# bluenote-1577/skani

Measured on AMD Instinct MI355X. Metric: genome-pairs/sec (triangle, ~5 Mbp genomes), higher is better.
Workload: dtype u64

## Files before the change

### skani_amd/csrc/capi.hip

```cpp
#include <algorithm>
#include <cmath>
#include <cstdlib>
#include <new>

#include "internal.h"

using namespace skh;

namespace {

template <class F> int guarded(skh_ctx* ctx, F&& f) {
    try {
        if (ctx) { PinScope scope(ctx->device, &ctx->ring); if (!ctx->pending_sorts.empty()) reap_pending_sorts(ctx); f(); } else f();
        return SKH_OK;
    }
    catch (const std::bad_alloc&) { if (ctx) ctx->err = "out of host memory"; return SKH_ERR_NOMEM; }
    catch (const PeerError& e) { if (ctx) ctx->err = e.what(); return SKH_ERR_PEER; }
    catch (const Error& e) { if (ctx) ctx->err = e.what(); return SKH_ERR_DEVICE; }
    catch (const std::invalid_argument& e) { if (ctx) ctx->err = e.what(); return SKH_ERR_INVALID; }
    catch (const std::exception& e) { if (ctx) ctx->err = e.what(); return SKH_ERR_INTERNAL; }
    catch (...) { if (ctx) ctx->err = "unknown error"; return SKH_ERR_INTERNAL; }
}

void check_params(const skh_sketch_params* p) {
// ... 38 lines not shown
    skh_ctx* ctx = new (std::nothrow) skh_ctx();
    if (!ctx) return SKH_ERR_NOMEM;
    int rc = guarded(ctx, [&] {
        dev_open(device, &ctx->stream, &ctx->stream2);
        ctx->device = device; ctx->ring.s0 = ctx->stream; ctx->ring.s1 = ctx->stream2;
        ctx->scan_ticket.alloc(2); dzero(ctx->scan_ticket.p, 8, ctx->stream); dsync(ctx->stream);
        auto env = [](const char* n, uint64_t dflt) { const char* v = getenv(n); return v && *v ? (uint64_t)strtoull(v, nullptr, 10) : dflt; };
        ctx->tune.seed_scratch_bytes = env("SKH_TUNE_SEED_SCRATCH_BYTES", ctx->tune.seed_scratch_bytes); ctx->tune.seed_scratch_fixed = getenv("SKH_TUNE_SEED_SCRATCH_BYTES") != nullptr;
        ctx->tune.seed_tile_cap = (uint32_t)env("SKH_TUNE_SEED_TILE_CAP", ctx->tune.seed_tile_cap);
        ctx->tune.screen_cells = env("SKH_TUNE_SCREEN_CELLS", ctx->tune.screen_cells);
        ctx->tune.chain_anchors = env("SKH_TUNE_CHAIN_ANCHORS", ctx->tune.chain_anchors);
        ctx->tune.chain_super_tiles = (uint32_t)env("SKH_TUNE_CHAIN_SUPER_TILES", ctx->tune.chain_super_tiles);
        ctx->tune.chain_dp_lds_slots = (uint32_t)env("SKH_TUNE_CHAIN_DP_LDS_SLOTS", ctx->tune.chain_dp_lds_slots);
        ctx->tune.build_match_cap = (uint32_t)env("SKH_TUNE_BUILD_MATCH_CAP", ctx->tune.build_match_cap);
        ctx->tune.marker_lds_max = (uint32_t)env("SKH_TUNE_MARKER_LDS_MAX", ctx->tune.marker_lds_max);
        ctx->tune.build_slice_max = (uint32_t)env("SKH_TUNE_BUILD_SLICE_MAX", ctx->tune.build_slice_max);
        ctx->tune.join_bitmap_words = (uint32_t)env("SKH_TUNE_JOIN_BITMAP_WORDS", ctx->tune.join_bitmap_words);
        ctx->tune.screen_planes = (uint32_t)env("SKH_TUNE_SCREEN_PLANES", ctx->tune.screen_planes);
        ctx->tune.screen_count_rows = (uint32_t)env("SKH_TUNE_SCREEN_COUNT_ROWS", ctx->tune.screen_count_rows);
        ctx->tune.screen_col_order = (uint32_t)env("SKH_TUNE_SCREEN_COL_ORDER", ctx->tune.screen_col_order);
        ctx->tune.marker_gate = (uint32_t)env("SKH_TUNE_MARKER_GATE", ctx->tune.marker_gate);
        ctx->tune.screen_cells_dense = (uint32_t)env("SKH_TUNE_SCREEN_CELLS_DENSE", 0);
        ctx->tune.build_resalt_all = (uint32_t)env("SKH_TUNE_BUILD_RESALT_ALL", 0);
        ctx->tune.screen_sort_radix = (uint32_t)env("SKH_TUNE_SCREEN_SORT_RADIX", 0);
        ctx->tune.skeys_avg = (uint32_t)env("SKH_TUNE_SKEYS_AVG", ctx->tune.skeys_avg);
        ctx->tune.skeys_cap = (uint32_t)env("SKH_TUNE_SKEYS_CAP", 0);
        ctx->tune.wide_sweep_dp = (uint32_t)env("SKH_TUNE_WIDE_SWEEP_DP", 0);
        ctx->tune.scan_one_max = env("SKH_TUNE_SCAN_ONE_MAX", ctx->tune.scan_one_max); ctx->tune.scan_two_max = env("SKH_TUNE_SCAN_TWO_MAX", ctx->tune.scan_two_max);
        ctx->tune.dist_fail = (uint32_t)env("SKH_TUNE_DIST_FAIL", 0);
        ctx->tune.dist_key_range_w1 = (uint32_t)env("SKH_TUNE_DIST_KEY_RANGE_W1", 0);
        ctx->tune.greedy_big_min = (uint32_t)env("SKH_TUNE_GREEDY_BIG_MIN", ctx->tune.greedy_big_min);
        ctx->tune.wide_span = std::min<uint64_t>(ctx->tune.wide_span, env("SKH_TUNE_WIDE_SPAN", ctx->tune.wide_span));
        ctx->tune.greedy_len_limit = (uint32_t)std::min<uint64_t>(0x10000, env("SKH_TUNE_GREEDY_LEN_LIMIT", 0x10000));
    });
    if (rc != SKH_OK) { delete ctx; return rc; }
    *out = ctx;
    return SKH_OK;
}

void skh_ctx_destroy(skh_ctx* ctx) {
    if (!ctx) return;
    dev_drain(ctx->device, ctx->stream, ctx->stream2);
    ctx->arena.release_all();
    ctx->model_c125 = GbdtModel(); ctx->model_c200 = GbdtModel(); ctx->scan_ticket.release(); ctx->part_cnt.release();
    dcache_trim();
    dev_close(ctx->stream, ctx->stream2);
    delete ctx;
}

const char* skh_last_error(const skh_ctx* ctx) { return ctx ? ctx->err.c_str() : "null context"; }
int skh_device_memory(uint64_t* live_bytes, uint64_t* idle_bytes, int trim) {
    try {
        if (trim) dcache_trim();
        size_t live = 0, idle = 0; dcache_stats(&live, &idle);
        if (live_bytes) *live_bytes = live;
        if (idle_bytes) *idle_bytes = idle;
        return SKH_OK;
    } catch (...) { return SKH_ERR_INTERNAL; }
}
void skh_free(void* p) { free(p); }

int skh_load_models(skh_ctx* ctx, const char* p125, const char* p200) {
    if (!ctx || !p125 || !p200) return SKH_ERR_INVALID;
    return guarded(ctx, [&] { load_model(ctx, p125, ctx->model_c125); load_model(ctx, p200, ctx->model_c200); });
}

int skh_genomes_pack(skh_ctx* ctx, const uint8_t* bases, const uint64_t* contig_off, const uint32_t* contig_genome, uint32_t n_contigs,
                     uint32_t n_genomes, int on_device, int seeding_mode, skh_genome_set** out) {
    if (!ctx || !out || (n_contigs && (!bases || !contig_off || !contig_genome))) return SKH_ERR_INVALID;
    *out = nullptr;
    skh_genome_set* gs = nullptr;
    int rc = guarded(ctx, [&] {
        if (seeding_mode != SKH_SEED_SCALAR && seeding_mode != SKH_SEED_AVX2) throw std::invalid_argument("bad seeding_mode");
        gs = new skh_genome_set();
        gs->ctx = ctx; gs->seeding_mode = seeding_mode;
        std::vector<uint64_t> len(n_contigs);
        for (uint32_t i = 0; i < n_contigs; i++) {
// ... 501 lines not shown
```

### skani_amd/csrc/chain.hip

```cpp
#include <algorithm>
#include <cmath>

#include "internal.h"

namespace skh {

#include "chain_types.h"
#include "chain_join.h"
#include "chain_chunk.h"
#include "chain_dp.h"
#include "chain_select.h"
#include "chain_stats.h"
#include "chain_estimate.h"

namespace {

static void genome_halves(const skh_sketch_set* S) {
    std::lock_guard<std::mutex> lk(S->cache_mu);
    if (S->halves.size() == S->n_genomes && S->n_genomes) return;
    S->halves.resize(S->n_genomes);
    for (uint32_t g = 0; g < S->n_genomes; g++) {
        skh_sketch_set::GenomeHalf& h = S->halves[g];
        h.n_pos = (uint32_t)(S->pos_off[g + 1] - S->pos_off[g]); h.pos0 = (uint32_t)S->pos_off[g];
        h.seed = S->p_seed.p + S->pos_off[g]; h.g = S->p_g.p + S->pos_off[g]; h.rep = S->p_rep.p; h.salt = S->salt[g];
// ... 301 lines not shown
                check_launch("chain_dp");
                SKH_LAUNCH(interval_emit_kernel<W>, (NC + 3) / 4, 256, 0, ctx->stream, NC, (const Chunk*)chunks, (const unsigned long long*)best,
                           (const uint32_t*)chunk_pair, ec);
                check_launch("interval_emit");
            }
        }
        if (!stage_filled) fill_regions(ctx, stage_fills);
#define SKH_GREEDY(CAP) SKH_LAUNCH(greedy_fast_kernel<CAP>, np, 64, 0, ctx->stream, np, (const uint32_t*)g_order, (const uint32_t*)d_pi0, (const uint32_t*)d_pc0, \
                   (const uint32_t*)ivl_cnt, (const Interval*)ivls, ctx->tune.greedy_len_limit, big_min, ivl_next, chunk_head, n_acc); check_launch("greedy_fast")
        tr.mark("dp (+order sort)");
        uint32_t* g_keys = ctx->arena.get<uint32_t>(np); uint32_t* g_order = ctx->arena.get<uint32_t>(np);
        if (np <= GREEDY_ORDER_ONE_MAX) {
            SKH_LAUNCH(greedy_order_kernel, 1u, 1024, 0, ctx->stream, np, (const uint32_t*)ivl_cnt, g_order);
            check_launch("greedy_order");
        } else {
            SKH_LAUNCH(greedy_order_keys_kernel, (np + 255) / 256, 256, 0, ctx->stream, np, (const uint32_t*)ivl_cnt, g_keys, g_order);
            check_launch("greedy_order_keys");
            sort_pairs_u32_u32(ctx, g_keys, g_order, np, 16);
        }
        SKH_GREEDY(256); SKH_GREEDY(512); SKH_GREEDY(1024);
#undef SKH_GREEDY
        SKH_LAUNCH(greedy_kernel, (np + 3) / 4, 256, 0, ctx->stream, np, (const uint32_t*)d_pi0, (const uint32_t*)d_pc0,
                   (const uint32_t*)ivl_cnt, (const Interval*)ivls, big_min, ivl_next, chunk_head, n_acc);
        check_launch("greedy");
        if (NS) {
            SKH_LAUNCH(greedy_big_kernel, np, 1024, 0, ctx->stream, np, (const uint32_t*)d_pi0, (const uint32_t*)d_ps0, (const uint32_t*)d_pc0,
                       (const uint32_t*)ivl_cnt, (const Interval*)ivls, big_min, greedy_scratch, ivl_next, chunk_head, n_acc);
            check_launch("greedy_big");
        }
        tr.mark("greedy");
        double* chunk_est = ctx->arena.get<double>(NC + 1); uint32_t* chunk_w = ctx->arena.get<uint32_t>(NC + 1);
        uint4* chunk_sums = ctx->arena.get<uint4>(NC + 1);
        if (NC) {
            SKH_LAUNCH(chunk_stats_kernel<W>, (NC + 255) / 256, 256, 0, ctx->stream, NC, (const Chunk*)chunks, (const uint32_t*)chunk_pair, (const uint32_t*)chunk_head,
                       (const uint32_t*)ivl_next, (const Interval*)ivls, d_pairs, d_wide, (const unsigned long long*)imk, c, k, chunk_est, chunk_w, chunk_sums);
            check_launch("chunk_stats");
        }
        tr.mark("chunk_stats");
        FinalizeArgs fa{};
        fa.n_pairs = np; fa.c = c; fa.k = k; fa.min_af = mp.min_af; fa.both_min_af = mp.both_min_af; fa.robust = mp.robust; fa.median = mp.median;
        fa.learned = model ? 1 : 0; fa.compute_ci = mp.compute_ci;
        if (model) { fa.nodes = model->nodes.p; fa.tree_off = model->off.p; fa.n_trees = model->n_trees; fa.shrinkage = model->shrinkage; fa.bias = model->bias; }
        FinalizeScratch fs{ctx->arena.get<double>(NC + 1), ctx->arena.get<double>(NC + 1), ctx->arena.get<uint32_t>(NC + 1), ctx->arena.get<uint32_t>(NC + 1),
                           ctx->arena.get<uint64_t>(NC + 1)};
        uint32_t* n_est = ctx->arena.get<uint32_t>(np);
#define SKH_FIN(CAP, MIN, MAX, THR) SKH_LAUNCH((finalize_kernel<CAP, MIN, MAX, THR>), np, THR, 0, ctx->stream, fa, d_pairs, (const uint32_t*)d_pc0, (const uint32_t*)n_chunks, \
                   (const double*)chunk_est, (const uint32_t*)chunk_w, (const uint4*)chunk_sums, fs, n_est, d_out + p0); \
        check_launch("finalize")
        bool any_mid = false, any_long = false;
        for (uint32_t i = 0; i < np && !any_long; i++) { any_mid = any_mid || pc0[i + 1] - pc0[i] > 320; any_long = pc0[i + 1] - pc0[i] > 1024; }
        SKH_FIN(320, 0, 320, FIN_THREADS);
        if (any_mid) { SKH_FIN(1024, 321, 1024, FIN_THREADS); }
        if (any_long) { SKH_FIN(1, 1025, 0xFFFFFFFFu, 1024); }
#undef SKH_FIN
        tr.mark("finalize");
        if (stats) {
            std::vector<uint32_t> h_nc(np), h_ni(np), h_nacc(np), h_ne(np);
            d2h(h_nc.data(), n_chunks, np * 4, ctx->stream); d2h(h_ni.data(), ivl_cnt, np * 4, ctx->stream);
            d2h(h_nacc.data(), n_acc, np * 4, ctx->stream); d2h(h_ne.data(), n_est, np * 4, ctx->stream);
            std::vector<Co> hanc((size_t)NA), hanr((size_t)NA);
            d2h(hanc.data(), anc_q, (uint64_t)NA * sizeof(Co), ctx->stream); d2h(hanr.data(), anc_r, (uint64_t)NA * sizeof(Co), ctx->stream);
            for (uint32_t i = 0; i < np; i++) {
                skh_chain_stats& st = stats[p0 + i];
                const uint32_t an = std::min(pair_anch[p0 + i], pa0[i + 1] - pa0[i]);
                st.switched = (pds[p0 + i].flags >> 2) & 1u; st.n_chunks = h_nc[i]; st.n_intervals = h_ni[i]; st.n_accepted = h_nacc[i]; st.n_estimates = h_ne[i];
                st.reserved = 0; st.n_anchors = pair_anch[p0 + i]; st.n_qpos = pair_inq[p0 + i];
                if constexpr (W::wide) st.anchor_checksum = an ? fnv_anchors(hanc, hanr, pa0[i], pa0[i] + an, job.host_go_a64[p0 + i], pds[p0 + i].a_nctg, job.host_go_b64[p0 + i], pds[p0 + i].b_nctg) : 0;
                else st.anchor_checksum = an ? fnv_anchors(hanc, hanr, pa0[i], pa0[i] + an, job.host_go_a[p0 + i], pds[p0 + i].a_nctg, job.host_go_b[p0 + i], pds[p0 + i].b_nctg) : 0;
                if (pair_anch[p0 + i] == 0) { st.switched = 1; st.n_qpos = 0; }
            }
        }
        if (ctx->pin_results.holds(out + p0)) d2h_pinned(out + p0, d_out + p0, (size_t)np * sizeof(skh_ani_result), ctx->stream);
        else d2h(out + p0, d_out + p0, (size_t)np * sizeof(skh_ani_result), ctx->stream);
        ctx->arena.rewind(arena_mark);
        p0 = p1;
        }
        ctx->arena.rewind(super_mark);
        sp0 = sp1;
    }
    uint32_t h_err = 0;
    d2h(&h_err, d_err, 4, ctx->stream);
    tr.mark("results d2h");
    if (h_err) throw Error("internal capacity bound violated in chain pipeline (" + std::to_string(h_err) + " events)");
}

}

// ... 118 lines not shown
```

### skani_amd/csrc/chain_estimate.h

```cpp
#pragma once

__device__ __forceinline__ double wave_sum_f64(double v) {
#pragma unroll
    for (int d = 32; d > 0; d >>= 1) v += __shfl_xor(v, d, 64);
    return v;
}
__device__ __forceinline__ uint64_t wave_sum_u64(uint64_t v) {
#pragma unroll
    for (int d = 32; d > 0; d >>= 1) v += __shfl_xor(v, d, 64);
    return v;
}

struct FinalizeArgs {
    uint32_t n_pairs, c, k;
    double min_af, both_min_af; int robust, median, learned, compute_ci;
    const GbdtModel::Node* nodes; const uint32_t* tree_off; uint32_t n_trees; float shrinkage, bias;
};
struct FinalizeScratch { double *u_est, *s_est; uint32_t *u_w, *s_w; uint64_t* cum; };

constexpr uint64_t WYRAND_STEP = 0xA0761D6478BD642Full;
__device__ __forceinline__ uint64_t wyrand_mix(uint64_t s) {
    const uint64_t b = s ^ 0xE7037ED1A0B428DBull;
    const uint32_t s0 = (uint32_t)s, s1 = (uint32_t)(s >> 32), b0 = (uint32_t)b, b1 = (uint32_t)(b >> 32);
    const uint64_t p00 = (uint64_t)s0 * b0;
    const uint64_t p01 = (uint64_t)s0 * b1 + (p00 >> 32);
    const uint64_t p10 = (uint64_t)s1 * b0 + (uint32_t)p01;
    const uint64_t p11 = (uint64_t)s1 * b1 + (p01 >> 32) + (p10 >> 32);
    return ((p10 << 32) | (uint32_t)p00) ^ p11;
}
__device__ __forceinline__ uint64_t wyrand_state(uint64_t d) { return 7ull + (d + 1ull) * WYRAND_STEP; }
__device__ __forceinline__ uint64_t wyrand_draw(uint64_t d) { return wyrand_mix(wyrand_state(d)); }

constexpr uint32_t FIN_WAVES = 2, FIN_THREADS = 64 * FIN_WAVES;
template <uint32_t FIN_LDS, uint32_t FIN_MIN, uint32_t FIN_MAX, uint32_t THREADS>
__global__ __launch_bounds__(THREADS) void finalize_kernel(FinalizeArgs fa, const PairDesc* pairs, const uint32_t* pc0, const uint32_t* n_chunks,
                                                       const double* chunk_est, const uint32_t* chunk_w, const uint4* chunk_sums, FinalizeScratch fs,
                                                       uint32_t* n_est_out, skh_ani_result* out) {
    __shared__ double lds_boot[128];
    __shared__ double lds_u[FIN_LDS], lds_s[FIN_LDS];
    __shared__ uint64_t lds_cum[FIN_LDS];
    __shared__ uint32_t lds_uw[FIN_LDS], lds_sw[FIN_LDS];
    __shared__ uint32_t lds_hdr[4];
    __shared__ uint64_t lds_total;
    const uint32_t wv = threadIdx.x >> 6, tid = threadIdx.x;
    const uint32_t p = blockIdx.x;
    if (p >= fa.n_pairs) return;
    const uint32_t l = lane_id();
    const PairDesc pd = pairs[p];
    const uint32_t C0 = pc0[p], nc = n_chunks[p];
    if (nc < FIN_MIN || nc > FIN_MAX) return;
    constexpr uint32_t WAVES = THREADS / 64;
    const bool in_lds = nc <= FIN_LDS;
    double* U = in_lds ? lds_u : fs.u_est + C0; uint32_t* UW = in_lds ? lds_uw : fs.u_w + C0;
    double* S = in_lds ? lds_s : fs.s_est + C0; uint32_t* SW = in_lds ? lds_sw : fs.s_w + C0;
    uint64_t* CUM = in_lds ? lds_cum : fs.cum + C0;
    if (wv == 0) {
        uint32_t n = 0, acl = 0, nchains = 0, tqb = 0;
        for (uint32_t b = 0; b < nc; b += 64) {
            const uint32_t s = C0 + b + l;
            if (b + l < nc) { const uint4 cs = chunk_sums[s]; acl += cs.x; nchains += cs.y; tqb += cs.z; }
            const bool v = b + l < nc && chunk_w[s] != NONE;
            const unsigned long long m = __ballot(v);
            if (v) { const uint32_t o = n + (uint32_t)__popcll(m & ((1ull << l) - 1ull)); U[o] = chunk_est[s]; UW[o] = chunk_w[s]; }
            n += (uint32_t)__popcll(m);
        }
        acl = wave_sum(acl); nchains = wave_sum(nchains); tqb = wave_sum(tqb);
        if (l == 0) { n_est_out[p] = n; lds_hdr[0] = n; lds_hdr[1] = acl; lds_hdr[2] = nchains; lds_hdr[3] = tqb; }
    }
    __syncthreads();
    const uint32_t n = lds_hdr[0], acl = lds_hdr[1], nchains = lds_hdr[2], tqb = lds_hdr[3];
// ... 59 lines not shown
        const uint64_t cv = i < n ? CUM[i] : 0;
        const unsigned long long mlo = __ballot(i < n && cv >= thr_lo), mhi = __ballot(i < n && cv >= thr_hi);
        if (lower_i == n && mlo) lower_i = b + (uint32_t)__ffsll((long long)mlo) - 1u;
        if (upper_i == n && mhi) upper_i = b + (uint32_t)__ffsll((long long)mhi) - 1u;
    }
    if (lower_i == n) lower_i = 0;
    upper_i = upper_i == n ? n - 1 : upper_i + 1;
    double wsum = 0., esum = 0.; uint64_t tm = 0;
    for (uint32_t i = l; i < n; i += 64) {
        const double e = S[i]; esum += e;
        if (i >= lower_i && i < upper_i) { wsum += e * (double)SW[i]; tm += SW[i]; }
    }
    wsum = wave_sum_f64(wsum); esum = wave_sum_f64(esum); tm = wave_sum_u64(tm);
    double final_ani = wsum / (double)tm;
    const double mean = esum / (double)n;
    double var = 0.;
    for (uint32_t i = l; i < n; i += 64) { const double d = mean - S[i]; var += d * d; }
    var = wave_sum_f64(var);
    const double sd = sqrt(var / (double)n);
    double ci_lo = 0., ci_hi = 1.;
    if (fa.compute_ci && n >= 10) {
        uint32_t nsteps = 0; while ((1u << nsteps) < n) nsteps++;
        auto search64 = [&](uint64_t x) { uint32_t lo = 0, hi = n - 1; for (uint32_t st = 0; st < nsteps; st++) { const uint32_t mid = (lo + hi) >> 1; const bool gt = CUM[mid] > x; hi = gt ? mid : hi; lo = gt ? lo : mid + 1; } return lo; };
        if (in_lds && total_mult < 0xFFFFFFFFull) {
            uint32_t* C32 = UW; uint32_t* T = (uint32_t*)U;
            uint32_t sh = 0; while ((total_mult >> sh) >= 512) sh++;
            const uint32_t nb = (uint32_t)(total_mult >> sh) + 1;
            for (uint32_t i = tid; i < n; i += THREADS) C32[i] = (uint32_t)CUM[i];
            for (uint32_t b = tid; b < nb; b += THREADS) T[b] = search64((uint64_t)b << sh) | (search64((uint64_t)(b + 1) << sh) << 16);
            __syncthreads();
            const uint32_t tot32 = (uint32_t)total_mult;
            const uint64_t step_it = (uint64_t)n * WYRAND_STEP, step_256 = 256ull * WYRAND_STEP;
            for (uint32_t it0 = 4 * wv; it0 < 100; it0 += 4 * WAVES) {
              uint64_t st[4];
#pragma unroll
              for (int u = 0; u < 4; u++) st[u] = wyrand_state((uint64_t)it0 * n + (uint64_t)l + 64u * (uint32_t)u);
              double sg[4];
#pragma unroll
              for (int g = 0; g < 4; g++) {
                double s = 0.;
                uint64_t sm[4];
#pragma unroll
                for (int u = 0; u < 4; u++) { sm[u] = st[u]; st[u] += step_it; }
                for (uint32_t j0 = l; j0 < n; j0 += 256) {
                    uint32_t x[4], lo[4], hi[4]; bool on[4];
#pragma unroll
                    for (int u = 0; u < 4; u++) {
                        const uint32_t j = j0 + 64u * (uint32_t)u;
                        on[u] = j < n;
                        const uint64_t r = wyrand_mix(sm[u]); sm[u] += step_256;
                        x[u] = (uint32_t)(((uint64_t)(uint32_t)(r >> 32) * tot32 + __umulhi((uint32_t)r, tot32)) >> 32);
                        const uint32_t tb = T[x[u] >> sh];
                        lo[u] = tb & 0xFFFFu; hi[u] = tb >> 16;
                    }
#pragma unroll
                    for (int u = 0; u < 4; u++) {
                        while (lo[u] < hi[u]) { const uint32_t mid = (lo[u] + hi[u]) >> 1; const bool gt = C32[mid] > x[u]; hi[u] = gt ? mid : hi[u]; lo[u] = gt ? lo[u] : mid + 1; }
                    }
#pragma unroll
                    for (int u = 0; u < 4; u++) if (on[u]) s += S[lo[u]];
                }
                sg[g] = s;
              }
#pragma unroll
              for (int d = 32; d > 0; d >>= 1) {
#pragma unroll
                  for (int g = 0; g < 4; g++) sg[g] += __shfl_xor(sg[g], d, 64);
              }
              if (l == 0) {
#pragma unroll
                  for (int g = 0; g < 4; g++) lds_boot[it0 + g] = sg[g] / (double)n;
              }
            }
        } else {
            for (uint32_t it = wv; it < 100; it += WAVES) {
                double s = 0.;
                for (uint32_t j0 = l; j0 < n; j0 += 64) {
                    const uint64_t r = wyrand_draw((uint64_t)it * n + j0);
                    s += S[search64(__umul64hi(r, total_mult))];
                }
                s = wave_sum_f64(s);
                if (l == 0) lds_boot[it] = s / (double)n;
            }
// ... 57 lines not shown
```

### skani_amd/csrc/chain_stats.h

```cpp
#pragma once

constexpr int STATS_REG = 4;

template <class W>
__global__ __launch_bounds__(256) void chunk_stats_kernel(uint32_t n_slots, const Chunk* chunks, const uint32_t* chunk_pair, const uint32_t* chunk_head,
                                                          const uint32_t* ivl_next, const Interval* ivls, const PairDesc* pairs, const WidePair* wide, const unsigned long long* inq_mask,
                                                          uint32_t c, uint32_t k, double* chunk_est, uint32_t* chunk_w, uint4* chunk_sums) {
    using Co = typename W::Co; using Arr = typename W::Arr;
    const uint32_t slot = blockIdx.x * blockDim.x + threadIdx.x;
    const uint32_t l = lane_id();
    const bool valid = slot < n_slots;
    const uint32_t head = valid ? chunk_head[slot] : NONE;
    if (valid) chunk_w[slot] = NONE;
    uint32_t total_anchors = 0, rq0 = 0xFFFFFFFFu, rq1 = 0, tbcq = 0, sum_len = 0, n_int = 0, s_begin = 0, s_end = 0; Co qoff = 0;
    uint32_t lo[STATS_REG], hi[STATS_REG];
#pragma unroll
    for (int i = 0; i < STATS_REG; i++) { lo[i] = 1; hi[i] = 0; }
    bool active = false;
    const void* ag = nullptr; uint32_t ag64 = 0; const unsigned long long* mk = nullptr;
    if (head != NONE) {
        const Chunk ck = chunks[slot];
        const uint32_t p = chunk_pair[slot];
        const bool switched = (pairs[p].flags & 4u) != 0;
        mk = inq_mask + (uint64_t)pairs[p].tile0 * (JOIN_TILE / 64);
        s_begin = ck.s_begin; s_end = ck.s_end;
        if constexpr (W::wide) { const CoArr a = wide[p].a_g; ag = a.p; ag64 = a.is64; qoff = wide[p].a_goff[ck.qctg]; }
        else { ag = pairs[p].a_g; qoff = ck.qoff; }
        for (uint32_t e = head; e != NONE; e = ivl_next[e]) {
            const Interval iv = ivls[e];
            total_anchors += iv.na;
            if (iv.q0 < rq0) rq0 = iv.q0;
            if (iv.q1 > rq1) rq1 = iv.q1;
            tbcq += (switched ? iv.r1 - iv.r0 : iv.q1 - iv.q0) + k + 2 * c;
            sum_len += (iv.q1 - iv.q0) + 2 * c + k;
            const uint32_t l0 = iv.q0 > c ? iv.q0 - c : 0, h0 = iv.q1 + c;
#pragma unroll
            for (int i = 0; i < STATS_REG; i++) if (n_int == (uint32_t)i) { lo[i] = l0; hi[i] = h0; }
            n_int++;
        }
        const bool sensitive = c < 200;
        active = rq1 - rq0 >= MIN_LENGTH_COVER;
        chunk_sums[slot] = make_uint4(sum_len, n_int, sensitive ? sum_len : (active ? rq1 - rq0 + 2 * c + k : 0u), 0u);
    } else if (valid) chunk_sums[slot] = make_uint4(0, 0, 0, 0);
    uint32_t in_u = 0, in_range = 0, in_list = 0;
    unsigned long long todo = __ballot(active);
    constexpr int PF = 4;
    struct Raw { Co v; unsigned long long m; };
    Raw cur[PF] = {}, nxt[PF] = {};
    auto fetch = [&](const Arr& ag_j, const unsigned long long* mk_j, uint32_t s2, uint32_t se_j) -> Raw {
        const uint32_t s = s2 < se_j ? s2 : (se_j ? se_j - 1u : 0u);
        const unsigned long long m = global_of(mk_j)[((s >> 8) << 2) | (s & 3u)];
        return Raw{(Co)ag_j[s], m};
    };
    auto value = [](const Raw& r, uint32_t s2, uint32_t se_j) -> Co {
        return s2 < se_j ? (r.v & ~(Co)1) | (Co)((r.m >> ((s2 >> 2) & 63u)) & 1ull) : (Co)0;
    };
    auto bcast_arr = [&](int src) -> Arr {
        const unsigned long long v = (unsigned long long)ag;
        const uint32_t lo32 = wave_readlane((uint32_t)v, src), hi32 = wave_readlane((uint32_t)(v >> 32), src);
        const void* ptr = (const void*)(((unsigned long long)hi32 << 32) | lo32);
        if constexpr (W::wide) return CoArr{ptr, wave_readlane(ag64, src)}; else return global_of((const uint32_t*)ptr);
    };
    auto bcast_ptr = [&](const void* ptr, int src) -> const void* {
        const unsigned long long v = (unsigned long long)ptr;
        const uint32_t lo32 = wave_readlane((uint32_t)v, src), hi32 = wave_readlane((uint32_t)(v >> 32), src);
        return (const void*)(((unsigned long long)hi32 << 32) | lo32);
    };
    int j = -1; uint32_t sb = 0, se = 0;
    Arr agj{}; const unsigned long long* mkj = nullptr;
    if (todo) {
        j = __ffsll((long long)todo) - 1; todo &= todo - 1ull;
        sb = wave_readlane(s_begin, j); se = wave_readlane(s_end, j);
        agj = bcast_arr(j); mkj = (const unsigned long long*)bcast_ptr(mk, j);
#pragma unroll
        for (int u = 0; u < PF; u++) cur[u] = fetch(agj, mkj, sb + 64u * (uint32_t)u + l, se);
    }
    while (j >= 0) {
        const bool more = todo != 0;
        const int jn = more ? __ffsll((long long)todo) - 1 : j;
        todo &= todo - 1ull;
        const uint32_t sbn = wave_readlane(s_begin, jn), sen = wave_readlane(s_end, jn);
        const Arr agn = bcast_arr(jn); const unsigned long long* mkn = (const unsigned long long*)bcast_ptr(mk, jn);
#pragma unroll
        for (int u = 0; u < PF; u++) nxt[u] = fetch(agn, mkn, sbn + 64u * (uint32_t)u + l, sen);
        const uint32_t nj = wave_readlane(n_int, j), q0j = wave_readlane(rq0, j), q1j = wave_readlane(rq1, j), headj = wave_readlane(head, j);
        const Co qoffj = wave_readlane(qoff, j);
        uint32_t lj[STATS_REG], wj[STATS_REG];
#pragma unroll
        for (int i = 0; i < STATS_REG; i++) { lj[i] = 0; wj[i] = 0; if (i == 0 || (uint32_t)i < nj) { lj[i] = wave_readlane(lo[i], j); wj[i] = wave_readlane(hi[i], j) - lj[i]; } }
        const uint32_t qwj = q1j - q0j;
        uint32_t cu = 0, cr = 0, cl = 0;
        auto count = [&](Co v) {
            const bool on = (v & 1u) != 0;
            const uint32_t pos = (uint32_t)((v >> 1) - qoffj);
            bool hit;
            if (nj <= (uint32_t)STATS_REG) {
                hit = pos - lj[0] <= wj[0];
                if (nj > 1) { hit = hit || pos - lj[1] <= wj[1]; if (nj > 2) { hit = hit || pos - lj[2] <= wj[2]; if (nj > 3) hit = hit || pos - lj[3] <= wj[3]; } }
            } else {
                hit = false;
                for (uint32_t e = headj; e != NONE; e = ivl_next[e]) { const Interval iv = ivls[e]; const uint32_t l0 = iv.q0 > c ? iv.q0 - c : 0; hit = hit || (pos >= l0 && pos <= iv.q1 + c); }
            }
            cl += (uint32_t)__popcll(__ballot(on));
            cu += (uint32_t)__popcll(__ballot(on && hit));
            cr += (uint32_t)__popcll(__ballot(on && pos - q0j <= qwj));
        };
#pragma unroll
        for (int u = 0; u < PF; u++) if (sb + 64u * (uint32_t)u < se) count(value(cur[u], sb + 64u * (uint32_t)u + l, se));
        for (uint32_t b2 = sb + 64u * PF; b2 < se; b2 += 64) count(value(fetch(agj, mkj, b2 + l, se), b2 + l, se));
        if ((int)l == j) { in_u = cu; in_range = cr; in_list = cl; }
        j = more ? jn : -1; sb = sbn; se = sen; agj = agn; mkj = mkn;
#pragma unroll
        for (int u = 0; u < PF; u++) cur[u] = nxt[u];
    }
    if (!active) return;
    uint32_t considered = in_list;
    const double inv_k = 1. / (double)k;
    const double putative = pow((double)total_anchors / (double)in_u, inv_k);
    if (putative > 0.950 && tbcq > c * 4 && rq1 - rq0 < CHUNK_SIZE * 9 / 10 && (double)considered > 1.05 * (double)in_range)
        considered = in_range;
    double ml = (double)total_anchors / (double)considered;
    if (!(ml < 1.)) ml = 1.;
    chunk_est[slot] = pow(ml, inv_k); chunk_w[slot] = considered;
}
```

### skani_amd/csrc/internal.h

```cpp
#pragma once
#include <chrono>
#include <functional>
#include <mutex>
#include <memory>
#include <string>
#include <vector>

#include "../../include/skani_hip.h"
#include "common.h"

namespace skh {

struct Arena {
    struct Chunk { char* p; size_t cap, off; };
    std::vector<Chunk> chunks;
    size_t min_chunk = (size_t)256 << 20;
    ~Arena() { for (auto& c : chunks) dfree(c.p); }
    void* take(size_t bytes) {
        bytes = (bytes + 255) & ~(size_t)255;
        for (auto& c : chunks) if (c.cap - c.off >= bytes) { void* r = c.p + c.off; c.off += bytes; return r; }
        size_t cap = bytes > min_chunk ? bytes : min_chunk;
        Chunk c{(char*)dmalloc(cap), cap, bytes};
        chunks.push_back(c);
        return c.p;
// ... 19 lines not shown
    DBuf<uint32_t> off; DBuf<Node> nodes;
    bool loaded() const { return n_trees != 0; }
};

}

struct skh_tunables {
    uint64_t seed_scratch_bytes = (uint64_t)16 << 30;
    bool seed_scratch_fixed = false;
    uint32_t seed_tile_cap = 0;
    uint64_t screen_cells = (uint64_t)2 << 30;
    uint64_t chain_anchors = (uint64_t)512 << 20;
    uint32_t chain_super_tiles = 1u << 20;
    uint32_t wide_sweep_dp = 0;
    uint32_t build_resalt_all = 0;
    uint32_t screen_sort_radix = 0;
    uint32_t skeys_avg = 1400;
    uint32_t skeys_cap = 0;
    uint32_t screen_cells_dense = 0;
    uint32_t screen_count_rows = 1;
    uint32_t screen_col_order = 1;
    uint32_t marker_gate = 1;
    uint32_t screen_planes = 8;
    uint32_t join_bitmap_words = 8192;
    uint32_t build_slice_max = 0;
    uint32_t marker_lds_max = 0;
    uint32_t build_match_cap = 0;
    uint32_t greedy_len_limit = 0x10000;
    uint32_t greedy_big_min = 2049;
    uint64_t scan_one_max = ~0ull, scan_two_max = ~0ull;
    uint32_t dist_key_range_w1 = 0;
    uint32_t dist_fail = 0;
    uint32_t chain_dp_lds_slots = 8;
    uint64_t wide_span = (1ull << 31) - 8192;
};

namespace skh {
struct PendingSort {
    DBuf<uint64_t> raw; DBuf<char> tmp; DevEvent ev; std::mutex mu;
    DBuf<uint32_t> mat; DBuf<uint64_t> work; DBuf<char> sort_tmp;
    void release() { std::lock_guard<std::mutex> lk(mu); raw.release(); tmp.release(); mat.release(); work.release(); sort_tmp.release(); }
};
}

struct skh_ctx {
    skh_tunables tune;
    int device = 0;
    devStream_t stream{};
    devStream_t stream2{};
    std::string err;
    skh::Arena arena;
    skh::GbdtModel model_c125, model_c200;
    skh_timings timings{};
    skh::PinBuf pin_pairs;
    skh::PinBuf pin_results;
    skh::PinRing ring;
    skh::DBuf<uint32_t> scan_ticket;
    bool screen_planes_checked = false;
    skh::DBuf<uint32_t> part_cnt; bool part_cnt_clean = false;
    std::vector<std::shared_ptr<skh::PendingSort>> pending_sorts;
};

namespace skh { struct Transport; }
struct skh_comm { skh::Transport* t = nullptr; ~skh_comm(); };

struct skh_genome_set {
    skh_ctx* ctx = nullptr;
    int seeding_mode = 0;
    uint32_t n_genomes = 0, n_contigs = 0;
    uint64_t n_words = 0, total_bases = 0;
    std::vector<skh::ContigDesc> contigs;
    std::vector<uint64_t> genome_contig_off;
    skh::DBuf<uint32_t> packed;
    skh::DBuf<uint32_t> nmask;
    skh::DBuf<skh::ContigDesc> d_contigs;
    std::vector<skh::SeedTile> tiles;
    std::vector<uint32_t> genome_first_tile;
    std::vector<uint32_t> tile_cached_for;
    skh::DBuf<skh::SeedTile> d_tiles;
    skh::DBuf<uint32_t> d_genome_first_tile;
    bool open = false; uint64_t cap_units = 0, n_units = 0; uint32_t cap_contigs = 0, n_batches = 0;
    skh::DBuf<uint8_t> stage[2];
    std::vector<std::shared_ptr<skh::DevEvent>> copied;
    std::mutex copied_mu;
};

struct skh_sketch_set {
    skh_ctx* ctx = nullptr;
    skh_sketch_params params{};
// ... 163 lines not shown
```

Before: 41.31 million.

## Count chunk stats via binary search and popcount; cache bootstrap draws in table

The chunk stats kernel gets a new default path. Each active lane finds the query-range and interval boundaries in its own sorted anchor list with galloping and binary searches, then counts marked anchors by popcounting mask words. This replaces the wave-cooperative streaming scan over every anchor, which remains available behind a tunable. Separately, the finalize bootstrap can read precomputed wyrand draws from a device table built once per context instead of hashing each draw, trading ALU work for global loads.

```diff
diff --git a/skani_amd/csrc/capi.hip b/skani_amd/csrc/capi.hip
--- a/skani_amd/csrc/capi.hip
+++ b/skani_amd/csrc/capi.hip
@@ -94,6 +94,8 @@
         ctx->tune.greedy_big_min = (uint32_t)env("SKH_TUNE_GREEDY_BIG_MIN", ctx->tune.greedy_big_min);
         ctx->tune.wide_span = std::min<uint64_t>(ctx->tune.wide_span, env("SKH_TUNE_WIDE_SPAN", ctx->tune.wide_span));
         ctx->tune.greedy_len_limit = (uint32_t)std::min<uint64_t>(0x10000, env("SKH_TUNE_GREEDY_LEN_LIMIT", 0x10000));
+        ctx->tune.stats_stream = (uint32_t)env("SKH_TUNE_STATS_STREAM", ctx->tune.stats_stream);
+        ctx->tune.boot_table = (uint32_t)env("SKH_TUNE_BOOT_TABLE", ctx->tune.boot_table);
     });
     if (rc != SKH_OK) { delete ctx; return rc; }
     *out = ctx;
@@ -104,7 +106,7 @@
     if (!ctx) return;
     dev_drain(ctx->device, ctx->stream, ctx->stream2);
     ctx->arena.release_all();
-    ctx->model_c125 = GbdtModel(); ctx->model_c200 = GbdtModel(); ctx->scan_ticket.release(); ctx->part_cnt.release();
+    ctx->model_c125 = GbdtModel(); ctx->model_c200 = GbdtModel(); ctx->scan_ticket.release(); ctx->part_cnt.release(); ctx->boot_draws.release();
     dcache_trim();
     dev_close(ctx->stream, ctx->stream2);
     delete ctx;
diff --git a/skani_amd/csrc/chain.hip b/skani_amd/csrc/chain.hip
--- a/skani_amd/csrc/chain.hip
+++ b/skani_amd/csrc/chain.hip
@@ -357,8 +357,10 @@
         double* chunk_est = ctx->arena.get<double>(NC + 1); uint32_t* chunk_w = ctx->arena.get<uint32_t>(NC + 1);
         uint4* chunk_sums = ctx->arena.get<uint4>(NC + 1);
         if (NC) {
-            SKH_LAUNCH(chunk_stats_kernel<W>, (NC + 255) / 256, 256, 0, ctx->stream, NC, (const Chunk*)chunks, (const uint32_t*)chunk_pair, (const uint32_t*)chunk_head,
-                       (const uint32_t*)ivl_next, (const Interval*)ivls, d_pairs, d_wide, (const unsigned long long*)imk, c, k, chunk_est, chunk_w, chunk_sums);
+#define SKH_STATS(STREAM) SKH_LAUNCH((chunk_stats_kernel<W, STREAM>), (NC + 255) / 256, 256, 0, ctx->stream, NC, (const Chunk*)chunks, (const uint32_t*)chunk_pair, (const uint32_t*)chunk_head, \
+                       (const uint32_t*)ivl_next, (const Interval*)ivls, d_pairs, d_wide, (const unsigned long long*)imk, c, k, chunk_est, chunk_w, chunk_sums)
+            if (ctx->tune.stats_stream) { SKH_STATS(true); } else { SKH_STATS(false); }
+#undef SKH_STATS
             check_launch("chunk_stats");
         }
         tr.mark("chunk_stats");
@@ -369,8 +371,14 @@
         FinalizeScratch fs{ctx->arena.get<double>(NC + 1), ctx->arena.get<double>(NC + 1), ctx->arena.get<uint32_t>(NC + 1), ctx->arena.get<uint32_t>(NC + 1),
                            ctx->arena.get<uint64_t>(NC + 1)};
         uint32_t* n_est = ctx->arena.get<uint32_t>(np);
-#define SKH_FIN(CAP, MIN, MAX, THR) SKH_LAUNCH((finalize_kernel<CAP, MIN, MAX, THR>), np, THR, 0, ctx->stream, fa, d_pairs, (const uint32_t*)d_pc0, (const uint32_t*)n_chunks, \
-                   (const double*)chunk_est, (const uint32_t*)chunk_w, (const uint4*)chunk_sums, fs, n_est, d_out + p0); \
+        if (ctx->tune.boot_table && fa.compute_ci && !ctx->boot_draws.p) {
+            ctx->boot_draws.alloc(BOOT_DRAWS);
+            SKH_LAUNCH(boot_draws_kernel, (BOOT_DRAWS + 255) / 256, 256, 0, ctx->stream, BOOT_DRAWS, ctx->boot_draws.p); check_launch("boot_draws");
+        }
+        const uint64_t* draws = ctx->tune.boot_table ? ctx->boot_draws.p : nullptr;
+#define SKH_FIN_T(CAP, MIN, MAX, THR, TAB) SKH_LAUNCH((finalize_kernel<CAP, MIN, MAX, THR, TAB>), np, THR, 0, ctx->stream, fa, d_pairs, (const uint32_t*)d_pc0, (const uint32_t*)n_chunks, \
+                   (const double*)chunk_est, (const uint32_t*)chunk_w, (const uint4*)chunk_sums, fs, draws, n_est, d_out + p0)
+#define SKH_FIN(CAP, MIN, MAX, THR) if (draws && CAP > 1) { SKH_FIN_T(CAP, MIN, MAX, THR, (CAP > 1)); } else { SKH_FIN_T(CAP, MIN, MAX, THR, false); } \
         check_launch("finalize")
         bool any_mid = false, any_long = false;
         for (uint32_t i = 0; i < np && !any_long; i++) { any_mid = any_mid || pc0[i + 1] - pc0[i] > 320; any_long = pc0[i + 1] - pc0[i] > 1024; }
@@ -378,6 +386,7 @@
         if (any_mid) { SKH_FIN(1024, 321, 1024, FIN_THREADS); }
         if (any_long) { SKH_FIN(1, 1025, 0xFFFFFFFFu, 1024); }
 #undef SKH_FIN
+#undef SKH_FIN_T
         tr.mark("finalize");
         if (stats) {
             std::vector<uint32_t> h_nc(np), h_ni(np), h_nacc(np), h_ne(np);
diff --git a/skani_amd/csrc/chain_estimate.h b/skani_amd/csrc/chain_estimate.h
--- a/skani_amd/csrc/chain_estimate.h
+++ b/skani_amd/csrc/chain_estimate.h
@@ -30,12 +30,18 @@
 }
 __device__ __forceinline__ uint64_t wyrand_state(uint64_t d) { return 7ull + (d + 1ull) * WYRAND_STEP; }
 __device__ __forceinline__ uint64_t wyrand_draw(uint64_t d) { return wyrand_mix(wyrand_state(d)); }
+constexpr uint32_t BOOT_RESAMPLES = 100, FIN_LDS_MAX = 1024, BOOT_DRAWS = BOOT_RESAMPLES * FIN_LDS_MAX;
+__global__ __launch_bounds__(256) void boot_draws_kernel(uint32_t n, uint64_t* table) {
+    const uint32_t d = blockIdx.x * blockDim.x + threadIdx.x;
+    if (d < n) table[d] = wyrand_draw(d);
+}
 
 constexpr uint32_t FIN_WAVES = 2, FIN_THREADS = 64 * FIN_WAVES;
-template <uint32_t FIN_LDS, uint32_t FIN_MIN, uint32_t FIN_MAX, uint32_t THREADS>
+template <uint32_t FIN_LDS, uint32_t FIN_MIN, uint32_t FIN_MAX, uint32_t THREADS, bool TABLE>
 __global__ __launch_bounds__(THREADS) void finalize_kernel(FinalizeArgs fa, const PairDesc* pairs, const uint32_t* pc0, const uint32_t* n_chunks,
                                                        const double* chunk_est, const uint32_t* chunk_w, const uint4* chunk_sums, FinalizeScratch fs,
-                                                       uint32_t* n_est_out, skh_ani_result* out) {
+                                                       const uint64_t* draws, uint32_t* n_est_out, skh_ani_result* out) {
+    static_assert(!TABLE || BOOT_RESAMPLES * FIN_LDS <= BOOT_DRAWS, "the draw table covers 100 resamples of the largest LDS instantiation");
     __shared__ double lds_boot[128];
     __shared__ double lds_u[FIN_LDS], lds_s[FIN_LDS];
     __shared__ uint64_t lds_cum[FIN_LDS];
@@ -161,9 +167,12 @@
             const uint32_t tot32 = (uint32_t)total_mult;
             const uint64_t step_it = (uint64_t)n * WYRAND_STEP, step_256 = 256ull * WYRAND_STEP;
             for (uint32_t it0 = 4 * wv; it0 < 100; it0 += 4 * WAVES) {
-              uint64_t st[4];
-#pragma unroll
-              for (int u = 0; u < 4; u++) st[u] = wyrand_state((uint64_t)it0 * n + (uint64_t)l + 64u * (uint32_t)u);
+              uint64_t st[4] = {};
+              if constexpr (!TABLE) {
+#pragma unroll
+                for (int u = 0; u < 4; u++) st[u] = wyrand_state((uint64_t)it0 * n + (uint64_t)l + 64u * (uint32_t)u);
+              }
+              const GlobalPtr<uint64_t> tab = global_of(draws);
               double sg[4];
 #pragma unroll
               for (int g = 0; g < 4; g++) {
@@ -171,13 +180,16 @@
                 uint64_t sm[4];
 #pragma unroll
                 for (int u = 0; u < 4; u++) { sm[u] = st[u]; st[u] += step_it; }
+                const uint32_t d0 = (it0 + (uint32_t)g) * n;
                 for (uint32_t j0 = l; j0 < n; j0 += 256) {
                     uint32_t x[4], lo[4], hi[4]; bool on[4];
 #pragma unroll
                     for (int u = 0; u < 4; u++) {
                         const uint32_t j = j0 + 64u * (uint32_t)u;
                         on[u] = j < n;
-                        const uint64_t r = wyrand_mix(sm[u]); sm[u] += step_256;
+                        uint64_t r;
+                        if constexpr (TABLE) r = on[u] ? tab[d0 + j] : 0ull;
+                        else { r = wyrand_mix(sm[u]); sm[u] += step_256; }
                         x[u] = (uint32_t)(((uint64_t)(uint32_t)(r >> 32) * tot32 + __umulhi((uint32_t)r, tot32)) >> 32);
                         const uint32_t tb = T[x[u] >> sh];
                         lo[u] = tb & 0xFFFFu; hi[u] = tb >> 16;
diff --git a/skani_amd/csrc/chain_stats.h b/skani_amd/csrc/chain_stats.h
--- a/skani_amd/csrc/chain_stats.h
+++ b/skani_amd/csrc/chain_stats.h
@@ -2,7 +2,7 @@
 
 constexpr int STATS_REG = 4;
 
-template <class W>
+template <class W, bool STREAM>
 __global__ __launch_bounds__(256) void chunk_stats_kernel(uint32_t n_slots, const Chunk* chunks, const uint32_t* chunk_pair, const uint32_t* chunk_head,
                                                           const uint32_t* ivl_next, const Interval* ivls, const PairDesc* pairs, const WidePair* wide, const unsigned long long* inq_mask,
                                                           uint32_t c, uint32_t k, double* chunk_est, uint32_t* chunk_w, uint4* chunk_sums) {
@@ -43,75 +43,168 @@
         chunk_sums[slot] = make_uint4(sum_len, n_int, sensitive ? sum_len : (active ? rq1 - rq0 + 2 * c + k : 0u), 0u);
     } else if (valid) chunk_sums[slot] = make_uint4(0, 0, 0, 0);
     uint32_t in_u = 0, in_range = 0, in_list = 0;
-    unsigned long long todo = __ballot(active);
-    constexpr int PF = 4;
-    struct Raw { Co v; unsigned long long m; };
-    Raw cur[PF] = {}, nxt[PF] = {};
-    auto fetch = [&](const Arr& ag_j, const unsigned long long* mk_j, uint32_t s2, uint32_t se_j) -> Raw {
-        const uint32_t s = s2 < se_j ? s2 : (se_j ? se_j - 1u : 0u);
-        const unsigned long long m = global_of(mk_j)[((s >> 8) << 2) | (s & 3u)];
-        return Raw{(Co)ag_j[s], m};
-    };
-    auto value = [](const Raw& r, uint32_t s2, uint32_t se_j) -> Co {
-        return s2 < se_j ? (r.v & ~(Co)1) | (Co)((r.m >> ((s2 >> 2) & 63u)) & 1ull) : (Co)0;
-    };
-    auto bcast_arr = [&](int src) -> Arr {
-        const unsigned long long v = (unsigned long long)ag;
-        const uint32_t lo32 = wave_readlane((uint32_t)v, src), hi32 = wave_readlane((uint32_t)(v >> 32), src);
-        const void* ptr = (const void*)(((unsigned long long)hi32 << 32) | lo32);
-        if constexpr (W::wide) return CoArr{ptr, wave_readlane(ag64, src)}; else return global_of((const uint32_t*)ptr);
-    };
-    auto bcast_ptr = [&](const void* ptr, int src) -> const void* {
-        const unsigned long long v = (unsigned long long)ptr;
-        const uint32_t lo32 = wave_readlane((uint32_t)v, src), hi32 = wave_readlane((uint32_t)(v >> 32), src);
-        return (const void*)(((unsigned long long)hi32 << 32) | lo32);
-    };
-    int j = -1; uint32_t sb = 0, se = 0;
-    Arr agj{}; const unsigned long long* mkj = nullptr;
-    if (todo) {
-        j = __ffsll((long long)todo) - 1; todo &= todo - 1ull;
-        sb = wave_readlane(s_begin, j); se = wave_readlane(s_end, j);
-        agj = bcast_arr(j); mkj = (const unsigned long long*)bcast_ptr(mk, j);
-#pragma unroll
-        for (int u = 0; u < PF; u++) cur[u] = fetch(agj, mkj, sb + 64u * (uint32_t)u + l, se);
-    }
-    while (j >= 0) {
-        const bool more = todo != 0;
-        const int jn = more ? __ffsll((long long)todo) - 1 : j;
-        todo &= todo - 1ull;
-        const uint32_t sbn = wave_readlane(s_begin, jn), sen = wave_readlane(s_end, jn);
-        const Arr agn = bcast_arr(jn); const unsigned long long* mkn = (const unsigned long long*)bcast_ptr(mk, jn);
-#pragma unroll
-        for (int u = 0; u < PF; u++) nxt[u] = fetch(agn, mkn, sbn + 64u * (uint32_t)u + l, sen);
-        const uint32_t nj = wave_readlane(n_int, j), q0j = wave_readlane(rq0, j), q1j = wave_readlane(rq1, j), headj = wave_readlane(head, j);
-        const Co qoffj = wave_readlane(qoff, j);
-        uint32_t lj[STATS_REG], wj[STATS_REG];
-#pragma unroll
-        for (int i = 0; i < STATS_REG; i++) { lj[i] = 0; wj[i] = 0; if (i == 0 || (uint32_t)i < nj) { lj[i] = wave_readlane(lo[i], j); wj[i] = wave_readlane(hi[i], j) - lj[i]; } }
-        const uint32_t qwj = q1j - q0j;
-        uint32_t cu = 0, cr = 0, cl = 0;
-        auto count = [&](Co v) {
-            const bool on = (v & 1u) != 0;
-            const uint32_t pos = (uint32_t)((v >> 1) - qoffj);
-            bool hit;
-            if (nj <= (uint32_t)STATS_REG) {
-                hit = pos - lj[0] <= wj[0];
-                if (nj > 1) { hit = hit || pos - lj[1] <= wj[1]; if (nj > 2) { hit = hit || pos - lj[2] <= wj[2]; if (nj > 3) hit = hit || pos - lj[3] <= wj[3]; } }
-            } else {
-                hit = false;
-                for (uint32_t e = headj; e != NONE; e = ivl_next[e]) { const Interval iv = ivls[e]; const uint32_t l0 = iv.q0 > c ? iv.q0 - c : 0; hit = hit || (pos >= l0 && pos <= iv.q1 + c); }
-            }
-            cl += (uint32_t)__popcll(__ballot(on));
-            cu += (uint32_t)__popcll(__ballot(on && hit));
-            cr += (uint32_t)__popcll(__ballot(on && pos - q0j <= qwj));
-        };
-#pragma unroll
-        for (int u = 0; u < PF; u++) if (sb + 64u * (uint32_t)u < se) count(value(cur[u], sb + 64u * (uint32_t)u + l, se));
-        for (uint32_t b2 = sb + 64u * PF; b2 < se; b2 += 64) count(value(fetch(agj, mkj, b2 + l, se), b2 + l, se));
-        if ((int)l == j) { in_u = cu; in_range = cr; in_list = cl; }
-        j = more ? jn : -1; sb = sbn; se = sen; agj = agn; mkj = mkn;
-#pragma unroll
-        for (int u = 0; u < PF; u++) cur[u] = nxt[u];
+    if constexpr (STREAM) {
+        unsigned long long todo = __ballot(active);
+        constexpr int PF = 4;
+        struct Raw { Co v; unsigned long long m; };
+        Raw cur[PF] = {}, nxt[PF] = {};
+        auto fetch = [&](const Arr& ag_j, const unsigned long long* mk_j, uint32_t s2, uint32_t se_j) -> Raw {
+            const uint32_t s = s2 < se_j ? s2 : (se_j ? se_j - 1u : 0u);
+            const unsigned long long m = global_of(mk_j)[((s >> 8) << 2) | (s & 3u)];
+            return Raw{(Co)ag_j[s], m};
+        };
+        auto value = [](const Raw& r, uint32_t s2, uint32_t se_j) -> Co {
+            return s2 < se_j ? (r.v & ~(Co)1) | (Co)((r.m >> ((s2 >> 2) & 63u)) & 1ull) : (Co)0;
+        };
+        auto bcast_arr = [&](int src) -> Arr {
+            const unsigned long long v = (unsigned long long)ag;
+            const uint32_t lo32 = wave_readlane((uint32_t)v, src), hi32 = wave_readlane((uint32_t)(v >> 32), src);
+            const void* ptr = (const void*)(((unsigned long long)hi32 << 32) | lo32);
+            if constexpr (W::wide) return CoArr{ptr, wave_readlane(ag64, src)}; else return global_of((const uint32_t*)ptr);
+        };
+        auto bcast_ptr = [&](const void* ptr, int src) -> const void* {
+            const unsigned long long v = (unsigned long long)ptr;
+            const uint32_t lo32 = wave_readlane((uint32_t)v, src), hi32 = wave_readlane((uint32_t)(v >> 32), src);
+            return (const void*)(((unsigned long long)hi32 << 32) | lo32);
+        };
+        int j = -1; uint32_t sb = 0, se = 0;
+        Arr agj{}; const unsigned long long* mkj = nullptr;
+        if (todo) {
+            j = __ffsll((long long)todo) - 1; todo &= todo - 1ull;
+            sb = wave_readlane(s_begin, j); se = wave_readlane(s_end, j);
+            agj = bcast_arr(j); mkj = (const unsigned long long*)bcast_ptr(mk, j);
+#pragma unroll
+            for (int u = 0; u < PF; u++) cur[u] = fetch(agj, mkj, sb + 64u * (uint32_t)u + l, se);
+        }
+        while (j >= 0) {
+            const bool more = todo != 0;
+            const int jn = more ? __ffsll((long long)todo) - 1 : j;
+            todo &= todo - 1ull;
+            const uint32_t sbn = wave_readlane(s_begin, jn), sen = wave_readlane(s_end, jn);
+            const Arr agn = bcast_arr(jn); const unsigned long long* mkn = (const unsigned long long*)bcast_ptr(mk, jn);
+#pragma unroll
+            for (int u = 0; u < PF; u++) nxt[u] = fetch(agn, mkn, sbn + 64u * (uint32_t)u + l, sen);
+            const uint32_t nj = wave_readlane(n_int, j), q0j = wave_readlane(rq0, j), q1j = wave_readlane(rq1, j), headj = wave_readlane(head, j);
+            const Co qoffj = wave_readlane(qoff, j);
+            uint32_t lj[STATS_REG], wj[STATS_REG];
+#pragma unroll
+            for (int i = 0; i < STATS_REG; i++) { lj[i] = 0; wj[i] = 0; if (i == 0 || (uint32_t)i < nj) { lj[i] = wave_readlane(lo[i], j); wj[i] = wave_readlane(hi[i], j) - lj[i]; } }
+            const uint32_t qwj = q1j - q0j;
+            uint32_t cu = 0, cr = 0, cl = 0;
+            auto count = [&](Co v) {
+                const bool on = (v & 1u) != 0;
+                const uint32_t pos = (uint32_t)((v >> 1) - qoffj);
+                bool hit;
+                if (nj <= (uint32_t)STATS_REG) {
+                    hit = pos - lj[0] <= wj[0];
+                    if (nj > 1) { hit = hit || pos - lj[1] <= wj[1]; if (nj > 2) { hit = hit || pos - lj[2] <= wj[2]; if (nj > 3) hit = hit || pos - lj[3] <= wj[3]; } }
+                } else {
+                    hit = false;
+                    for (uint32_t e = headj; e != NONE; e = ivl_next[e]) { const Interval iv = ivls[e]; const uint32_t l0 = iv.q0 > c ? iv.q0 - c : 0; hit = hit || (pos >= l0 && pos <= iv.q1 + c); }
+                }
+                cl += (uint32_t)__popcll(__ballot(on));
+                cu += (uint32_t)__popcll(__ballot(on && hit));
+                cr += (uint32_t)__popcll(__ballot(on && pos - q0j <= qwj));
+            };
+#pragma unroll
+            for (int u = 0; u < PF; u++) if (sb + 64u * (uint32_t)u < se) count(value(cur[u], sb + 64u * (uint32_t)u + l, se));
+            for (uint32_t b2 = sb + 64u * PF; b2 < se; b2 += 64) count(value(fetch(agj, mkj, b2 + l, se), b2 + l, se));
+            if ((int)l == j) { in_u = cu; in_range = cr; in_list = cl; }
+            j = more ? jn : -1; sb = sbn; se = sen; agj = agn; mkj = mkn;
+#pragma unroll
+            for (int u = 0; u < PF; u++) cur[u] = nxt[u];
+        }
+    } else if (active) {
+        Arr arr{};
+        if constexpr (W::wide) arr = CoArr{ag, ag64}; else arr = global_of((const uint32_t*)ag);
+        const auto mkg = global_of(mk);
+        const uint32_t sb = s_begin, se = s_end > s_begin ? s_end : s_begin;
+        auto pos_at = [&](uint32_t s) -> uint32_t { return (uint32_t)((Co)(arr[s] >> 1) - qoff); };
+        uint32_t r0 = sb, r1 = sb;
+        {
+            uint32_t h0 = se, h1 = se, st0 = 1, st1 = 1;
+            while (r0 < h0 || r1 < h1) {
+                const bool o0 = r0 < h0, o1 = r1 < h1;
+                uint32_t m0 = r0 + ((h0 - r0) >> 1), m1 = r1 + ((h1 - r1) >> 1);
+                if (st0) m0 = h0 - r0 > st0 ? r0 + (st0 - 1u) : h0 - 1u;
+                if (st1) m1 = h1 - r1 > st1 ? h1 - st1 : r1;
+                const uint32_t p0 = o0 ? pos_at(m0) : 0u, p1 = o1 ? pos_at(m1) : 0u;
+                if (o0) { if (p0 >= rq0) { h0 = m0; st0 = 0; } else { r0 = m0 + 1; st0 <<= 1; } }
+                if (o1) { if (p1 > rq1) { h1 = m1; st1 <<= 1; } else { r1 = m1 + 1; st1 = 0; } }
+            }
+        }
+        uint32_t ia[STATS_REG], ib[STATS_REG];
+#pragma unroll
+        for (int i = 0; i < STATS_REG; i++) { ia[i] = sb; ib[i] = sb; }
+        if (n_int == 1) {
+            uint32_t a = r0, b = r1; bool ga = true, gb = true;
+            while (ga || gb) {
+                ga = ga && a > sb; gb = gb && b < se;
+                const uint32_t pa = ga ? pos_at(a - 1) : 0u, pb = gb ? pos_at(b) : 0u;
+                ga = ga && pa >= lo[0]; gb = gb && pb <= hi[0];
+                a -= ga ? 1u : 0u; b += gb ? 1u : 0u;
+            }
+            ia[0] = a; ib[0] = b;
+        } else if (n_int <= (uint32_t)STATS_REG) {
+            uint32_t L[STATS_REG], H[STATS_REG];
+#pragma unroll
+            for (int i = 0; i < STATS_REG; i++) { const bool on = (uint32_t)i < n_int; L[i] = on ? lo[i] : 0xFFFFFFFFu; H[i] = on ? hi[i] : 0u; }
+            auto cx = [&](int x, int y) { if (L[y] < L[x]) { const uint32_t tl = L[x], th = H[x]; L[x] = L[y]; H[x] = H[y]; L[y] = tl; H[y] = th; } };
+            cx(0, 1); cx(2, 3); cx(0, 2); cx(1, 3); cx(1, 2);
+            static_assert(STATS_REG == 4, "the sorting network above is for four intervals");
+            uint32_t ah[STATS_REG], bh[STATS_REG];
+#pragma unroll
+            for (int i = 0; i < STATS_REG; i++) {
+                const bool on = (uint32_t)i < n_int;
+                if (on && L[i] > rq0) ia[i] = r0;
+                ah[i] = on ? (L[i] <= rq0 ? r0 : r1) : sb;
+                if (on) ib[i] = H[i] >= rq1 ? r1 : r0;
+                bh[i] = on ? (H[i] >= rq1 ? se : r1) : sb;
+            }
+            for (;;) {
+                bool open = false;
+                uint32_t pa[STATS_REG], pb[STATS_REG];
+#pragma unroll
+                for (int i = 0; i < STATS_REG; i++) {
+                    const bool oa = ia[i] < ah[i], ob = ib[i] < bh[i];
+                    open = open || oa || ob;
+                    pa[i] = oa ? pos_at(ia[i] + ((ah[i] - ia[i]) >> 1)) : 0u; pb[i] = ob ? pos_at(ib[i] + ((bh[i] - ib[i]) >> 1)) : 0u;
+                }
+                if (!open) break;
+#pragma unroll
+                for (int i = 0; i < STATS_REG; i++) {
+                    if (ia[i] < ah[i]) { const uint32_t m = ia[i] + ((ah[i] - ia[i]) >> 1); if (pa[i] >= L[i]) ah[i] = m; else ia[i] = m + 1; }
+                    if (ib[i] < bh[i]) { const uint32_t m = ib[i] + ((bh[i] - ib[i]) >> 1); if (pb[i] > H[i]) bh[i] = m; else ib[i] = m + 1; }
+                }
+            }
+            uint32_t done = sb;
+#pragma unroll
+            for (int i = 0; i < STATS_REG; i++) { if (ia[i] < done) ia[i] = done; if (ib[i] > done) done = ib[i]; }
+        } else {
+            for (uint32_t s = sb; s < se; s++) {
+                if (!((mkg[((s >> 8) << 2) | (s & 3u)] >> ((s >> 2) & 63u)) & 1ull)) continue;
+                const uint32_t pos = pos_at(s);
+                bool hit = false;
+                for (uint32_t e = head; e != NONE; e = ivl_next[e]) { const Interval iv = ivls[e]; const uint32_t l0 = iv.q0 > c ? iv.q0 - c : 0; hit = hit || (pos >= l0 && pos <= iv.q1 + c); }
+                in_u += hit ? 1u : 0u;
+            }
+        }
+        for (uint32_t base = sb & ~255u; base < se; base += 256) {
+            unsigned long long w[4];
+#pragma unroll
+            for (uint32_t r = 0; r < 4; r++) w[r] = mkg[(base >> 6) | r];
+            auto below = [&](uint32_t s) -> uint32_t {
+                const uint32_t x = s <= base ? 0u : (s - base < 256u ? s - base : 256u);
+                uint32_t n = 0;
+#pragma unroll
+                for (uint32_t r = 0; r < 4; r++) { const uint32_t nb = (x + 3u - r) >> 2; n += (uint32_t)__popcll(w[r] & (nb >= 64u ? ~0ull : (1ull << nb) - 1ull)); }
+                return n;
+            };
+            in_list += below(se) - below(sb);
+            in_range += below(r1) - below(r0);
+#pragma unroll
+            for (int i = 0; i < STATS_REG; i++) if (ib[i] > ia[i]) in_u += below(ib[i]) - below(ia[i]);
+        }
     }
     if (!active) return;
     uint32_t considered = in_list;
diff --git a/skani_amd/csrc/internal.h b/skani_amd/csrc/internal.h
--- a/skani_amd/csrc/internal.h
+++ b/skani_amd/csrc/internal.h
@@ -75,6 +75,8 @@
     uint32_t dist_key_range_w1 = 0;
     uint32_t dist_fail = 0;
     uint32_t chain_dp_lds_slots = 8;
+    uint32_t stats_stream = 0;
+    uint32_t boot_table = 1;
     uint64_t wide_span = (1ull << 31) - 8192;
 };
 
@@ -98,6 +100,7 @@
     skh::PinBuf pin_pairs;
     skh::PinBuf pin_results;
     skh::PinRing ring;
+    skh::DBuf<uint64_t> boot_draws;
     skh::DBuf<uint32_t> scan_ticket;
     bool screen_planes_checked = false;
     skh::DBuf<uint32_t> part_cnt; bool part_cnt_clean = false;
```

After: 41.59 million, median of 6. About the same (+0.7%).
